# tpoisonooo/how-to-optimize-gemm

Measured on AMD Instinct MI355X. Metric: GFLOPS vs N (square SGEMM sweep); % of MI355X fp32 MFMA peak at N=4096, higher is better.
Workload: dtype f32; 1 GPU; sgemm fp32 square N=4096, 1xMI355X, kernel=auto (BASELINE configs[2]); m=4096, n=4096, k=4096, kernel=MMult_hip_auto, parallelism=single, rows_per_rank=4096

## Files before the change

### how-to-optimize-gemm_amd/csrc/abi.hip

```cpp
#include <algorithm>

#include "internal.hpp"
#include "igemm_plan.hpp"
#ifdef MMH_AB_BUILD
#include "ab_kernels.hpp"
#endif

using namespace mmh;

namespace {
template <typename F>
int time_calls(mmh_context *h, void *stream, int warmup, int reps, float *ms_per_call, const char *what, F call) {
  if (!h || reps <= 0 || warmup < 0 || !ms_per_call) return MMH_ERR_INVALID_ARG;
  ENTER(h);
  hipStream_t s = static_cast<hipStream_t>(stream);
  int rc = MMH_OK;
  for (int i = 0; i < warmup && rc == MMH_OK; ++i) rc = call(s);
  if (rc != MMH_OK) return rc;
  hipEvent_t t0 = nullptr, t1 = nullptr;
  hipError_t e = hipEventCreate(&t0);
  if (e == hipSuccess) e = hipEventCreate(&t1);
  if (e == hipSuccess) e = hipEventRecord(t0, s);
  for (int i = 0; i < reps && rc == MMH_OK && e == hipSuccess; ++i) rc = call(s);
  float ms = 0.f;
// ... 41 lines not shown
  return time_calls(h, stream, warmup, reps, ms_per_call, what, [&](hipStream_t s) {
    c.g.s = s;
    return call_on(h, c.call, h->kernel, c.g, c.b);
  });
}

constexpr KernelRow kKernels[] = {
    {MMH_KERNEL_AUTO, "MMult_hip_auto", Launcher::Auto, -1},
    {MMH_KERNEL_VALU, "MMult_hip_valu", Launcher::Valu, -1},
    {MMH_KERNEL_VALU_128X128, "MMult_hip_valu_128x128", Launcher::Valu, -1},
    {MMH_KERNEL_VALU_64X64, "MMult_hip_valu_64x64", Launcher::Valu, -1},
    {MMH_KERNEL_VALU_128X64, "MMult_hip_valu_128x64", Launcher::Valu, -1},
    {MMH_KERNEL_MFMA, "MMult_hip_mfma", Launcher::Reg, -1},
    {MMH_KERNEL_MFMA_256, "MMult_hip_mfma256", Launcher::Reg, -1},
    {MMH_KERNEL_NAIVE, "MMult_hip_naive", Launcher::Naive, -1},
    {MMH_KERNEL_MFMA_SIMPLE, "MMult_hip_mfma_simple", Launcher::Reg, -1},
    {MMH_KERNEL_MFMA_PIPE, "MMult_hip_mfma_pipe", Launcher::Reg, -1},
    {MMH_KERNEL_MFMA_TILES, "MMult_hip_mfma_tiles", Launcher::Reg, -1},
    {MMH_KERNEL_MFMA_128X64, "MMult_hip_mfma_128x64", Launcher::Reg, -1},
    {MMH_KERNEL_MFMA_64X64, "MMult_hip_mfma_64x64", Launcher::Reg, -1},
    {MMH_KERNEL_MFMA_256X256, "MMult_hip_mfma_256x256", Launcher::Reg, -1},
    {MMH_KERNEL_MFMA_64X64_DMA, "MMult_hip_mfma_64x64_dma", Launcher::K2L, MMH_KERNEL_MFMA_64X64},
    {MMH_KERNEL_MFMA_128X64_DMA, "MMult_hip_mfma_128x64_dma", Launcher::K2L, MMH_KERNEL_MFMA_128X64},
    {MMH_KERNEL_MFMA_128X128_DMA, "MMult_hip_mfma_128x128_dma", Launcher::K2L, MMH_KERNEL_MFMA},
    {MMH_KERNEL_MFMA_64X64_DMA5, "MMult_hip_mfma_64x64_dma5", Launcher::K2W, MMH_KERNEL_MFMA_64X64},
    {MMH_KERNEL_MFMA_128X64_DMA5, "MMult_hip_mfma_128x64_dma5", Launcher::K2W, MMH_KERNEL_MFMA_128X64},
    {MMH_KERNEL_MFMA_128X128_DMA5, "MMult_hip_mfma_128x128_dma5", Launcher::K2W, MMH_KERNEL_MFMA},
    {MMH_KERNEL_MFMA_96X96_DMA5, "MMult_hip_mfma_96x96_dma5", Launcher::K2W, MMH_KERNEL_MFMA},
    {MMH_KERNEL_MFMA_96X64_DMA5, "MMult_hip_mfma_96x64_dma5", Launcher::K2W, MMH_KERNEL_MFMA},
    {MMH_KERNEL_MFMA_160X160_DMA5, "MMult_hip_mfma_160x160_dma5", Launcher::K2W, MMH_KERNEL_MFMA},
    {MMH_KERNEL_MFMA_SPLITK, "MMult_hip_mfma_splitk", Launcher::SplitK, MMH_KERNEL_MFMA},
    {MMH_KERNEL_MFMA_SPLITK_128X64, "MMult_hip_mfma_splitk_128x64", Launcher::SplitK, MMH_KERNEL_MFMA_128X64},
#ifdef MMH_AB_BUILD
#include "ab_kernels.inc"
#endif
};
constexpr int kMaxKernelId = 127;
struct KernelIndex {
  signed char row[kMaxKernelId + 1];
  bool ok;
};
constexpr KernelIndex kernel_index() {
  KernelIndex ix{};
  ix.ok = true;
  for (signed char &r : ix.row) r = -1;
  int n = 0;
  for (const KernelRow &r : kKernels) {
    if (r.id < 0 || r.id > kMaxKernelId || ix.row[r.id] >= 0) ix.ok = false;
    else ix.row[r.id] = (signed char)n;
    ++n;
  }
  for (const KernelRow &r : kKernels)
    if (r.fallback >= 0 && (ix.row[r.fallback] < 0 || kKernels[ix.row[r.fallback]].launcher != Launcher::Reg)) ix.ok = false;
  return ix;
}
constexpr KernelIndex kKernelIndex = kernel_index();
static_assert(kKernelIndex.ok, "kKernels: an id twice or out of range, or a fall-back that is no register-staged id");

struct OptionRow {
  int id;
  int mmh_context::*field;
  int lo, hi;
  bool squash;
};
constexpr OptionRow kOptions[] = {
    {MMH_OPT_STREAMK, &mmh_context::streamk, 0, 2, false},
    {MMH_OPT_SPLITK, &mmh_context::splitk, 0, 16, false},
    {MMH_OPT_HOST_PANELS, &mmh_context::host_panels, -1, kMaxHostPanels, false},
    {MMH_OPT_STREAMK_ORDER, &mmh_context::sk_order, 0, 1, true},
    {MMH_OPT_STREAMK_CHAIN, &mmh_context::sk_chain, 0, 1, true},
    {MMH_OPT_PERSIST, &mmh_context::persist, 0, 1, false},
    {MMH_OPT_RIM, &mmh_context::rim, 0, kAbBuild ? 16 : 0, false},
    {MMH_OPT_RIM5, &mmh_context::rim5, 0, 0, kAbBuild},
#ifdef MMH_AB_BUILD
    {100, &mmh_context::pin, 0, 1, true},
    {101, &mmh_context::ab_group_m, 0, 1024, false},
    {102, &mmh_context::ab_nodefer, 0, 1, true},
    {103, &mmh_context::ab_own_occ, 0, 1, true},
    {104, &mmh_context::sk_order_min10, 10, 1000, false},
    {105, &mmh_context::ab_valu_old, 0, 1, true},
    {106, &mmh_context::ab_whole_ranges, 0, 1, true},
    {107, &mmh_context::split_tail, 0, 1, true},
    {108, &mmh_context::ab_batch_major, 0, 1, true},
#endif
};
const OptionRow *option_row(int option) {
  for (const OptionRow &r : kOptions)
    if (r.id == option) return &r;
  return nullptr;
}
}

const KernelRow *mmh::kernel_row(int kernel) {
  if (kernel < 0 || kernel > kMaxKernelId || kKernelIndex.row[kernel] < 0) return nullptr;
  return &kKernels[kKernelIndex.row[kernel]];
}

extern "C" {

const char *mmh_strerror(int status) {
  switch (status) {
    case MMH_OK: return "success";
    case MMH_ERR_INVALID_ARG: return "invalid argument";
    case MMH_ERR_HIP: return "HIP runtime error";
    case MMH_ERR_NO_DEVICE: return "no gfx950 device";
    case MMH_ERR_UNSUPPORTED: return "unsupported in this build";
    case MMH_ERR_ALLOC: return "allocation failed";
    case MMH_ERR_COMM: return "RCCL error";
    default: return "unknown status";
  }
}

const char *mmh_last_error(void) { return last_error_ref().c_str(); }

const char *mmh_last_launch(void) { return last_launch_ref().c_str(); }

int mmh_version(void) { return 303; }

int mmh_is_ab_build(void) {
#ifdef MMH_AB_BUILD
  return 1;
#else
  return 0;
#endif
}

int mmh_device_count(int *count) {
  if (!count) return MMH_ERR_INVALID_ARG;
  int c = 0;
  hipError_t e = hipGetDeviceCount(&c);
  if (e != hipSuccess) {
    *count = 0;
    (void)hipGetLastError();
    return MMH_OK;
  }
  *count = c;
  return MMH_OK;
}

int mmh_device_info(int device, char *name, int *cu_count, int *clock_mhz) {
  hipDeviceProp_t prop;
  HIP_TRY(hipGetDeviceProperties(&prop, device));
  if (name) snprintf(name, 256, "%s (%s)", prop.name, prop.gcnArchName);
  if (cu_count) *cu_count = prop.multiProcessorCount;
  if (clock_mhz) *clock_mhz = prop.clockRate / 1000;
  return MMH_OK;
}

int mmh_create(mmh_handle_t *handle, int device) {
  if (!handle) return MMH_ERR_INVALID_ARG;
  return create_context(handle, device);
}

int mmh_destroy(mmh_handle_t h) {
  destroy_context(h);
  return MMH_OK;
}

int mmh_set_kernel(mmh_handle_t h, int kernel) {
  if (!h || !known_kernel(kernel)) return MMH_ERR_INVALID_ARG;
  h->kernel = kernel;
  return MMH_OK;
}

int mmh_set_option(mmh_handle_t h, int option, int value) {
  if (!h) return MMH_ERR_INVALID_ARG;
// ... 240 lines not shown
```

### how-to-optimize-gemm_amd/csrc/internal.hpp

```cpp
#pragma once
#include <hip/hip_runtime.h>
#include <stdint.h>
#include <stdio.h>
#include <string.h>

#include <initializer_list>
#include <string>
#include <utility>
#include <vector>

#include "ab_build.hpp"
#include "../../include/mmult_hip.h"

namespace mmh {

void set_last_error(const std::string &s);
void set_last_launch(const std::string &s);
const std::string &last_error_ref();
const std::string &last_launch_ref();
int hip_fail(hipError_t e, const char *what);

#define HIP_TRY(expr)                                        \
  do {                                                       \
    hipError_t e_ = (expr);                                  \
// ... 27 lines not shown
struct GemmArgs {
  int m, n, k;
  const float *A;
  int lda;
  const float *B;
  int ldb;
  float *C;
  int ldc;
  int acc;
  hipStream_t s;
  int rim_m = 0, rim_n = 0;
  int form = 0;
  int sk_w = 0;
  int ta = 0, tb = 0;
  int ex = 0;
  float alpha = 1.0f, beta = 0.0f;
  const float *bias = nullptr;
  int bias_mode = MMH_BIAS_NONE, act = MMH_ACT_NONE;
};
inline GemmArgs op_args(int ta, int tb, int m, int n, int k, const float *dA, int lda, const float *dB, int ldb, float *dC, int ldc,
                        int accumulate, hipStream_t s) {
  GemmArgs g{m, n, k, dA, lda, dB, ldb, dC, ldc, accumulate ? 1 : 0, s};
  g.ta = ta;
  g.tb = tb;
  return g;
}
inline GemmArgs ex_args_of(GemmArgs g, float alpha, float beta, const float *dBias, int bias_mode, int activation) {
  g.acc = 0;
  g.ex = 1;
  g.alpha = alpha;
  g.beta = beta;
  g.bias = dBias;
  g.bias_mode = bias_mode;
  g.act = activation;
  return g;
}

}

struct mmh_context {
  int device = 0;
  int kernel = MMH_KERNEL_AUTO;
  int cu_count = 0;
  mmh::DevBuf a, b, c;
  mmh::Scratch bt;
  int igemm_mode = 0;
  int i8_grid_cap = 0;
  mmh::Scratch qa, qb, qc, qs;
  void *qs_zeros_of = nullptr;
  mmh::Scratch colsum_parts;
  struct StreamWs {
    hipStream_t stream = nullptr;
    mmh::DevBuf flags;
    bool flags_dirty = true;
    mmh::DevBuf parts;
    unsigned long stamp = 0;
    bool captured = false;
  };
  std::vector<StreamWs *> ws;
  unsigned long ws_stamp = 0;
  int *sk_stats = nullptr;
  std::vector<void *> retired;
  int streamk = 1;
  int splitk = 0;
  int host_panels = -1;
  void *rocblas = nullptr;
  void *blaslt = nullptr;
  int *sticky = nullptr;
  int *sticky_dev = nullptr;
  long long spin_limit = 1ll << 26;
  int fault = 0;
  int pin = 1;
  int sk_order = 1;
  int sk_order_min10 = 18;
  int dma_edge = 1;
  int dma_dword_rows = 1;
  int sk_chain = 1;
  int rim5 = 0;
  int ab_whole_ranges = 0;
  int ab_nodefer = 0;
  int ab_valu_old = 0;
  int ab_own_occ = 0;
  int split_tail = 1;
  int ab_group_m = 0;
  int ab_batch_major = 0;
  int persist = 0;
  int rim = 0;
  struct SkTable {
    long tiles = 0;
    int nk = 0, grid = 0;
    mmh::DevBuf buf;
    int *host = nullptr;
    size_t host_ints = 0;
    unsigned long stamp = 0;
    bool pinned = false;
    bool uploaded = false;
    std::vector<hipStream_t> upload_streams;
  };
  std::vector<SkTable *> sk_tables;
  unsigned long sk_stamp = 0;
  std::vector<std::pair<const void *, int>> per_cu;
  bool warmed = false;
  hipStream_t hs_in = nullptr, hs_run = nullptr, hs_out = nullptr;
  hipEvent_t ev_in[mmh::kMaxHostPanels] = {}, ev_run[mmh::kMaxHostPanels] = {}, ev_b = nullptr;
  bool pipeline_ready = false;
  hipEvent_t t0 = nullptr, t1 = nullptr;
};

namespace mmh {

int check_sticky(mmh_context *h);
#define ENTER(h)                                       \
  ::mmh::DeviceGuard guard_;                           \
  HIP_TRY(guard_.enter((h)->device));                  \
  if (int st_ = ::mmh::check_sticky(h); st_ != MMH_OK) return st_

int create_context(mmh_context **out, int device, bool warm = true);
void destroy_context(mmh_context *h);
int warm_context(mmh_context *h);

inline bool aligned16(const void *p) { return (reinterpret_cast<uintptr_t>(p) & 15) == 0; }
inline bool capturing(hipStream_t s) {
  hipStreamCaptureStatus cap = hipStreamCaptureStatusNone;
  (void)hipStreamIsCapturing(s, &cap);
  return cap != hipStreamCaptureStatusNone;
}

inline bool fast_shape(int BM, int BN, int KB, const GemmArgs &g) {
  return (g.m % BM == 0) && (g.n % BN == 0) && (g.k % KB == 0) && (g.lda % 4 == 0) && (g.ldb % 4 == 0) &&
         (g.ldc % 4 == 0) && aligned16(g.A) && aligned16(g.B) && aligned16(g.C);
}
inline bool window_ok(int BM, int BN, int k, int lda, int ldb) {
  const size_t lim = (1ull << 31) - 4096;
  return ((size_t)BM * lda + k) * 4 < lim && ((size_t)k * ldb + BN) * 4 < lim;
}
inline bool window_ok(int BM, int BN, const GemmArgs &g) {
  if (!g.ta && !g.tb) return window_ok(BM, BN, g.k, g.lda, g.ldb);
  const size_t lim = (1ull << 31) - 4096;
  const size_t a = g.ta ? (size_t)g.k * g.lda + BM : (size_t)BM * g.lda + g.k;
  const size_t b = g.tb ? (size_t)BN * g.ldb + g.k : (size_t)g.k * g.ldb + BN;
  return a * 4 < lim && b * 4 < lim;
}

int check_gemm_args(int m, int n, int k, const void *A, int lda, const void *B, int ldb, const void *C, int ldc, int ta = 0,
                    int tb = 0);

enum class Launcher { Auto, Valu, Naive, Reg, SplitK, K2L, K2W, K2M  };
struct KernelRow {
  int id;
  const char *name;
  Launcher launcher;
  int fallback;
};
const KernelRow *kernel_row(int kernel);
inline bool known_kernel(int kernel) { return kernel_row(kernel) != nullptr; }
inline bool is_family(int kernel, Launcher l) {
  const KernelRow *r = kernel_row(kernel);
  return r && r->launcher == l;
}

int workspace_for(mmh_context *ctx, hipStream_t s, long tiles, size_t parts_bytes, int **flags, float **parts);
int reserve_stream(mmh_context *ctx, hipStream_t s, int m, int n, int k);
void workspaces_suspect(mmh_context *ctx);
int reserve_scratch(mmh_context *ctx, hipStream_t s, const char *who, std::initializer_list<ScratchNeed> needs);
bool build_sk_tables(long tiles, int nk, int grid, int *order, int *place);
int sk_tables_for(mmh_context *ctx, long tiles, int nk, int grid, hipStream_t s, const int **order, const int **place, int min10 = 0);

int auto_plan(int m, int n, int k, int lda, int ldb, int ldc, int base_align, int cu_count, int *kernel, long *tiles,
              int *streamk_grid);
int sgemm_on(mmh_context *ctx, int kernel, int m, int n, int k, const float *dA, int lda, const float *dB, int ldb,
             float *dC, int ldc, int accumulate, hipStream_t s);
int auto_plan_op(int ta, int tb, int m, int n, int k, int lda, int ldb, int ldc, int base_align, int cu_count, int *kernel,
                 long *tiles, int *streamk_grid, int ex = 0);
int launch_reg(mmh_context *ctx, int kernel, const GemmArgs &g);
int launch_reg_splitk(mmh_context *ctx, int tile , int S, const GemmArgs &g);
int warm_reg(mmh_context *ctx, float *scratch, hipStream_t s);
int launch_dma(mmh_context *ctx, int kernel, const GemmArgs &g);
bool dma_shape_ok(const mmh_context *ctx, int kernel, const GemmArgs &g);
int warm_dma(mmh_context *ctx, float *scratch, hipStream_t s);
int launch_dma32(mmh_context *ctx, int kernel, const GemmArgs &g);
bool dma32_shape_ok(const mmh_context *ctx, int kernel, const GemmArgs &g);
int warm_dma32(mmh_context *ctx, float *scratch, hipStream_t s);
inline bool dma5_tail_split(long tiles, long w, long cus, int k) {
  const long rem = tiles - w * cus;
  return w >= 2 && k >= 512 && 100 * rem > 85 * cus && rem <= cus && (w * cus) % 8 == 0;
}

inline bool dma5_rim_dims(int m, int n, int *r_m, int *r_n) {
  const int rm = m % 64, rn = n % 64;
  const int a = (rm == 1 && m > 64) ? 1 : 0, b = (rn == 1 && n > 64) ? 1 : 0;
  if (r_m) *r_m = a;
  if (r_n) *r_n = b;
  return a > 0 || b > 0;
}
template <class... Tile>
struct TileTable {
  template <class F>
  static int with(int kernel, F &&f, int none) {
    int r = none;
    (void)((kernel == Tile::ID && ((r = f(Tile{})), true)) || ...);
    return r;
  }
  template <class F>
  static int each(F &&f) {
    int rc = MMH_OK;
    (void)(((rc = f(Tile{})) == MMH_OK) && ...);
    return rc;
  }
};

template <int ID_, int BM_, int BN_, int WTN_, int WTM_, int KB_>
struct RegTile {
  static constexpr int ID = ID_, BM = BM_, BN = BN_, WTN = WTN_, WTM = WTM_, KB = KB_;
};
using reg_tiles = TileTable<
    RegTile<MMH_KERNEL_MFMA,         128, 128, 4, 4, 32>,
    RegTile<MMH_KERNEL_MFMA_256X256, 256, 256, 4, 8, 32>,
    RegTile<MMH_KERNEL_MFMA_128X64,  128, 64,  2, 4, 32>,
    RegTile<MMH_KERNEL_MFMA_64X64,   64,  64,  2, 2, 128>>;
inline long reg_tile_count(int kernel, int m, int n) {
  long tiles = 0;
  reg_tiles::with(kernel, [&](auto t) {
    tiles = (long)((m + t.BM - 1) / t.BM) * ((n + t.BN - 1) / t.BN);
    return 0;
  }, 0);
  return tiles;
}

template <int ID_, int BM_, int BN_, int KB_, int WTM_, int WTN_, int NBUF_>
struct K2lTile {
  static constexpr int ID = ID_, BM = BM_, BN = BN_, KB = KB_, WTM = WTM_, WTN = WTN_, NBUF = NBUF_;
};
using k2l_tiles = TileTable<
    K2lTile<MMH_KERNEL_MFMA_64X64_DMA,   64,  64,  32, 2, 2, 3>,
    K2lTile<MMH_KERNEL_MFMA_128X64_DMA,  128, 64,  32, 4, 2, 3>,
    K2lTile<MMH_KERNEL_MFMA_128X128_DMA, 128, 128, 32, 4, 4, 3>>;

template <int ID_, int BM_, int BN_, int WTM_, int WTN_, int NBUF_, int NL_, int D_, bool SK_, bool OPS_, int RS_ = 1>
struct K2wTile {
  static constexpr int ID = ID_, BM = BM_, BN = BN_, WTM = WTM_, WTN = WTN_, NBUF = NBUF_, NL = NL_, D = D_, RS = RS_;
  static constexpr bool SK = SK_, OPS = OPS_;
};
#define MMH_K2W_ARGS(K) K::BM, K::BN, 32, K::WTM, K::WTN, K::NBUF
using k2w_tiles = TileTable<
    K2wTile<MMH_KERNEL_MFMA_64X64_DMA5,   64,  64, 2, 2, 3, 2, 2, true,  true>,
    K2wTile<MMH_KERNEL_MFMA_128X64_DMA5,  128, 64, 4, 2, 3, 4, 2, true,  true>,
    K2wTile<MMH_KERNEL_MFMA_128X128_DMA5, 128, 128, 4, 4, 3, 4, 2, true, true>,
    K2wTile<MMH_KERNEL_MFMA_96X96_DMA5,   96,  96, 3, 3, 3, 1, 2, false, false>,
    K2wTile<MMH_KERNEL_MFMA_160X160_DMA5, 160, 160, 5, 5, 3, 4, 2, false, false>,
    K2wTile<MMH_KERNEL_MFMA_96X64_DMA5,   96,  64, 3, 2, 3, 4, 2, false, false>>;

struct BatchArgs {
  long long sA = 0, sB = 0, sC = 0;
  long batch = 1;
  long long sBias = 0;
};
constexpr long kBatchedMaxWorkgroups = MMH_BATCHED_MAX_WORKGROUPS;

inline int dma5_form(const mmh_context *ctx, int BM, int BN, const GemmArgs &g, const BatchArgs &b = BatchArgs{}) {
  if (!window_ok(BM, BN, g)) return -1;
  const bool s4 = b.batch == 1 || (b.sA % 4 == 0 && b.sB % 4 == 0 && b.sC % 4 == 0);
  if (fast_shape(BM, BN, 32, g) && s4) return 0;
  if (!ctx || !ctx->dma_edge) return -1;
  const bool rows16 = (g.lda % 4 == 0) && (g.ldb % 4 == 0) && aligned16(g.A) && aligned16(g.B) &&
                      (b.batch == 1 || (b.sA % 4 == 0 && b.sB % 4 == 0));
  if (!rows16 && !ctx->dma_dword_rows) return -1;
  return 1;
}
// ... 51 lines not shown
```

### how-to-optimize-gemm_amd/csrc/launch_dma5.hpp

```cpp
#pragma once
#include <stdarg.h>

#include <tuple>

#include "ab_build.hpp"
#include "launch_common.hpp"
#include "sgemm_dma5.hpp"

namespace mmh {

inline const char *op_tag(const GemmArgs &g) {
  return g.ta ? (g.tb ? ", operands TT" : ", operands TN") : (g.tb ? ", operands NT" : "");
}
inline std::string ex_tag(const GemmArgs &g) {
  std::string t = std::string(g.ta ? (g.tb ? ", operands TT" : ", operands TN") : (g.tb ? ", operands NT" : ", operands NN")) + ", epilogue";
  const size_t bare = t.size();
  if (g.alpha != 1.0f) t += " alpha";
  if (g.beta != 0.0f) t += " beta";
  if (g.bias_mode == MMH_BIAS_COL) t += " bias(col)";
  if (g.bias_mode == MMH_BIAS_ROW) t += " bias(row)";
  if (g.act == MMH_ACT_RELU) t += " relu";
  if (t.size() == bare) t += " identity";
  return t;
}
inline Dma5Epilogue ex_args(const GemmArgs &g) { return Dma5Epilogue{g.alpha, g.beta, g.bias, g.bias_mode, g.act}; }

template <typename K>
long dma5_split_first(mmh_context *ctx, K twin, int threads, size_t lds, long tiles, int k) {
  if (!ctx || !ctx->split_tail) return tiles;
  (void)allow_big_lds(twin, lds);
  const long cus = ctx->cu_count > 0 ? ctx->cu_count : 256;
  const long w = std::min(resident_per_cu(ctx, twin, threads, lds), 3);
  return dma5_tail_split(tiles, w, cus, k) ? w * cus : tiles;
}

template <class K_>
struct NnForm {
  using K = K_;
  static constexpr bool NN = true, SK = K::SK;
  static constexpr const char *plain_name = "sgemm_mfma_dma5_kernel", *streamk_name = "sgemm_dma5_streamk_kernel";
  static auto plain(bool edge) {
    return edge ? sgemm_mfma_dma5_kernel<MMH_K2W_ARGS(K), true, K::NL, K::D, K::RS>
                : sgemm_mfma_dma5_kernel<MMH_K2W_ARGS(K), false, K::NL, K::D, K::RS>;
  }
  static auto streamk_bound() { return sgemm_dma5_streamk_kernel<MMH_K2W_ARGS(K), true, true, K::NL, K::D, K::RS>; }
  static auto streamk(bool edge, bool chained) {
    return edge ? (chained ? streamk_bound() : sgemm_dma5_streamk_kernel<MMH_K2W_ARGS(K), true, false, K::NL, K::D, K::RS>)
                : (chained ? sgemm_dma5_streamk_kernel<MMH_K2W_ARGS(K), false, true, K::NL, K::D, K::RS>
                           : sgemm_dma5_streamk_kernel<MMH_K2W_ARGS(K), false, false, K::NL, K::D, K::RS>);
  }
  static std::string tag(const GemmArgs &) { return {}; }
  static std::tuple<> extra(const GemmArgs &) { return {}; }
  static int acc(const mmh_context *ctx, const GemmArgs &g) {
    if (kAbBuild && ctx) return g.acc | (ctx->ab_nodefer ? 2 : 0) | (ctx->ab_whole_ranges ? 4 : 0) | ((ctx->ab_group_m & 0xff) << 8);
    return g.acc;
  }
};
template <class K_, int OP>
struct OpForm {
  using K = K_;
  static constexpr bool NN = false, SK = K::SK;
  static constexpr const char *plain_name = "sgemm_mfma_dma5_op_kernel", *streamk_name = "sgemm_dma5_op_streamk_kernel";
  static auto plain(bool edge) {
    return edge ? sgemm_mfma_dma5_op_kernel<MMH_K2W_ARGS(K), true, K::NL, K::D, OP>
                : sgemm_mfma_dma5_op_kernel<MMH_K2W_ARGS(K), false, K::NL, K::D, OP>;
  }
  static auto streamk(bool edge, bool) {
    return edge ? sgemm_dma5_op_streamk_kernel<MMH_K2W_ARGS(K), true, K::NL, K::D, OP>
                : sgemm_dma5_op_streamk_kernel<MMH_K2W_ARGS(K), false, K::NL, K::D, OP>;
  }
  static std::string tag(const GemmArgs &g) { return op_tag(g); }
  static std::tuple<> extra(const GemmArgs &) { return {}; }
  static int acc(const mmh_context *, const GemmArgs &g) { return g.acc; }
};
template <class K_, int OP>
struct ExForm {
  using K = K_;
  static constexpr bool NN = false, SK = K::SK;
  static constexpr const char *plain_name = "sgemm_mfma_dma5_ex_kernel", *streamk_name = "sgemm_dma5_ex_streamk_kernel";
  static auto plain(bool edge) {
    return edge ? sgemm_mfma_dma5_ex_kernel<MMH_K2W_ARGS(K), true, K::NL, K::D, OP>
                : sgemm_mfma_dma5_ex_kernel<MMH_K2W_ARGS(K), false, K::NL, K::D, OP>;
  }
  static auto streamk(bool edge, bool) {
    return edge ? sgemm_dma5_ex_streamk_kernel<MMH_K2W_ARGS(K), true, K::NL, K::D, OP>
                : sgemm_dma5_ex_streamk_kernel<MMH_K2W_ARGS(K), false, K::NL, K::D, OP>;
  }
  static std::string tag(const GemmArgs &g) { return ex_tag(g); }
  static std::tuple<Dma5Epilogue> extra(const GemmArgs &g) { return {ex_args(g)}; }
  static int acc(const mmh_context *, const GemmArgs &) { return 0; }
};

template <class K_, int OP>
struct BatchedForm {
  using K = K_;
  static constexpr bool SK = false;
  static constexpr const char *plain_name = "sgemm_mfma_dma5_batched_kernel";
  static auto plain(bool edge) {
    return edge ? sgemm_mfma_dma5_batched_kernel<MMH_K2W_ARGS(K), true, K::NL, K::D, OP>
                : sgemm_mfma_dma5_batched_kernel<MMH_K2W_ARGS(K), false, K::NL, K::D, OP>;
  }
  static std::string tag(const GemmArgs &g) { return op_tag(g); }
  static std::tuple<int> front(const mmh_context *ctx, const GemmArgs &g) {
    return {g.acc | ((kAbBuild && ctx && ctx->ab_batch_major) ? 2 : 0)};
  }
  static std::tuple<> back(const GemmArgs &, const BatchArgs &, long) { return {}; }
};
inline std::tuple<Dma5Epilogue, long long> ex_chunk_args(const GemmArgs &g, const BatchArgs &bt, long b0) {
  const bool none = g.bias_mode == MMH_BIAS_NONE;
  Dma5Epilogue ep = ex_args(g);
  ep.bias = none ? nullptr : g.bias + b0 * bt.sBias;
  return {ep, none ? 0 : bt.sBias};
}
template <class K_, int OP>
struct BatchedExForm {
  using K = K_;
  static constexpr bool SK = false;
  static constexpr const char *plain_name = "sgemm_mfma_dma5_batched_ex_kernel";
  static auto plain(bool edge) {
    return edge ? sgemm_mfma_dma5_batched_ex_kernel<MMH_K2W_ARGS(K), true, K::NL, K::D, OP>
                : sgemm_mfma_dma5_batched_ex_kernel<MMH_K2W_ARGS(K), false, K::NL, K::D, OP>;
  }
  static std::string tag(const GemmArgs &g) { return ex_tag(g); }
  static std::tuple<> front(const mmh_context *, const GemmArgs &) { return {}; }
  static std::tuple<Dma5Epilogue, long long> back(const GemmArgs &g, const BatchArgs &bt, long b0) { return ex_chunk_args(g, bt, b0); }
};

constexpr int kTextSize = 448;
inline int text_add(char *what, int at, const char *format, ...) __attribute__((format(printf, 3, 4)));
inline int text_add(char *what, int at, const char *format, ...) {
  va_list args;
  va_start(args, format);
  const int n = vsnprintf(what + at, kTextSize - at, format, args);
  va_end(args);
  return std::min(at + std::max(n, 0), kTextSize - 1);
}
template <class K>
int dma5_tile_text(char *what, const char *kernel) {
  return text_add(what, 0, "%s<%d,%d> wave tile %dx%d, K-slice %d x %d ring buffers by %d loader wave%s' LDS-DMA, fragments %d k-steps ahead",
                  kernel, K::BM, K::BN, 16 * K::WTM, 16 * K::WTN, 32, K::NBUF, K::NL, K::NL > 1 ? "s" : "", K::D);
}
template <class K>
int dma5_plain_text(char *what, const char *kernel, bool edge, long workgroups, bool split) {
  return text_add(what, dma5_tile_text<K>(what, kernel), ", %s%ld workgroups of %d threads%s", edge ? "guarded, " : "", workgroups,
                  Dma5Tile<MMH_K2W_ARGS(K), K::NL>::THREADS, split ? " (the last round as a launch of its own)" : "");
}
template <class L>
void dma5_launch_rounds(long first, long tiles, L launch) {
  launch(first, 0L);
  if (first < tiles) launch(tiles - first, first);
}

template <class F>
int launch_dma5_tile(mmh_context *ctx, const GemmArgs &g) {
  using K = typename F::K;
  constexpr int BM = K::BM, BN = K::BN, KB = 32;
  using T = Dma5Tile<MMH_K2W_ARGS(K), K::NL>;
  const int form = dma5_form(ctx, BM, BN, g);
  if (form < 0) return 1;
  const bool edge = form == 1;
  GemmArgs ga = g;
  ga.acc = F::acc(ctx, g);
  if constexpr (F::SK) {
    if (ctx && ctx->streamk) {
      const bool chained = !F::NN || ctx->sk_chain != 0;
      auto occ = NnForm<K>::streamk_bound();
      auto kern = F::streamk(edge, chained);
      if constexpr (F::NN) {
        if (kAbBuild && ctx->ab_own_occ && !edge) occ = kern;
      } else {
        (void)allow_big_lds(occ, T::LDS_BYTES);
      }
      char what[kTextSize];
      text_add(what, dma5_tile_text<K>(what, F::streamk_name), "%s%s", chained ? ", chained parts" : "", edge ? ", guarded" : "");
      const int order_min10 = (BM == 128 && BN == 128) ? 10 : 0;
      const int sk = std::apply([&](auto... x) {
        return launch_streamk(ctx, kern, occ, BM, BN, KB, T::THREADS, T::LDS_BYTES, what, ga, full_tiles(g.m, g.n, BM, BN), order_min10, x...);
      }, F::extra(g));
      if (!F::NN && sk == MMH_OK) set_last_launch(last_launch_ref() + F::tag(g));
      if (sk <= 0) return sk;
    }
  }
  const int nbm = (g.m + BM - 1) / BM, nbn = (g.n + BN - 1) / BN;
  const long tiles = (long)nbm * nbn;
  const long first = dma5_split_first(ctx, NnForm<K>::plain(edge), T::THREADS, T::LDS_BYTES, tiles, g.k);
  const int acc_bits = edge ? F::acc(nullptr, g) : ga.acc;
  auto kern = F::plain(edge);
  const int ok = allow_big_lds(kern, T::LDS_BYTES);
  if (ok != MMH_OK) return ok;
  dma5_launch_rounds(first, tiles, [&](long workgroups, long id0) {
    std::apply([&](auto... x) {
      hipLaunchKernelGGL(kern, dim3((unsigned)workgroups), dim3(T::THREADS), T::LDS_BYTES, g.s, g.m, g.n, g.k, g.A, g.lda, g.B, g.ldb, g.C,
                         g.ldc, acc_bits | (int)((unsigned)(id0 >> 3) << 16), nbm, nbn, x...);
    }, F::extra(g));
  });
  HIP_TRY(hipGetLastError());
  char what[kTextSize];
  text_add(what, dma5_plain_text<K>(what, F::plain_name, edge, tiles, first < tiles), "%s", F::tag(g).c_str());
  set_last_launch(what);
  return MMH_OK;
}

template <class F>
int launch_batched_tile(mmh_context *ctx, const GemmArgs &g, const BatchArgs &bt) {
  using K = typename F::K;
  using T = Dma5Tile<MMH_K2W_ARGS(K), K::NL>;
  const int form = dma5_form(ctx, K::BM, K::BN, g, bt);
  if (form < 0) return 1;
  const bool edge = form == 1;
  auto kern = F::plain(edge);
  const int ok = allow_big_lds(kern, T::LDS_BYTES);
  if (ok != MMH_OK) return ok;
  const int nbm = (g.m + K::BM - 1) / K::BM, nbn = (g.n + K::BN - 1) / K::BN;
  const long per = (long)nbm * nbn;
  const long mats = std::max(1L, kBatchedMaxWorkgroups / per);
  long launches = 0;
  bool split = false;
  for (long b0 = 0; b0 < bt.batch; b0 += mats) {
    const long tiles = std::min(mats, bt.batch - b0) * per;
    const float *A = g.A + b0 * bt.sA, *B = g.B + b0 * bt.sB;
    float *C = g.C + b0 * bt.sC;
    const long first = dma5_split_first(ctx, NnForm<K>::plain(edge), T::THREADS, T::LDS_BYTES, tiles, g.k);
    dma5_launch_rounds(first, tiles, [&](long workgroups, long id0) {
      std::apply([&](auto... x) {
        hipLaunchKernelGGL(kern, dim3((unsigned)workgroups), dim3(T::THREADS), T::LDS_BYTES, g.s, g.m, g.n, g.k, A, g.lda, bt.sA, B, g.ldb,
                           bt.sB, C, g.ldc, bt.sC, x...);
      }, std::tuple_cat(F::front(ctx, g), std::make_tuple(nbm, nbn, (unsigned)id0), F::back(g, bt, b0)));
      ++launches;
    });
    split |= first < tiles;
    HIP_TRY(hipGetLastError());
  }
  char what[kTextSize];
  int at = dma5_plain_text<K>(what, F::plain_name, edge, bt.batch * per, split);
  at = text_add(what, at, "%s, batch %ld", F::tag(g).c_str(), bt.batch);
  if (launches > 1) text_add(what, at, " as %ld launches", launches);
  set_last_launch(what);
  return MMH_OK;
}

template <class L>
int launch_naive_chunks(const GemmArgs &g, const BatchArgs &b, std::string what, L launch) {
  const long gx = (g.n + 63) / 64, gy = (g.m + 3) / 4;
  const long mats = std::max(1L, std::min(65535L, kBatchedMaxWorkgroups / (gx * gy)));
  long launches = 0;
  for (long b0 = 0; b0 < b.batch; b0 += mats) {
    launch(dim3((unsigned)gx, (unsigned)gy, (unsigned)std::min(mats, b.batch - b0)), g.A ? g.A + b0 * b.sA : nullptr,
           g.B ? g.B + b0 * b.sB : nullptr, g.C + b0 * b.sC, b0);
    ++launches;
    HIP_TRY(hipGetLastError());
  }
  what += ", batch " + std::to_string(b.batch);
  if (launches > 1) what += " as " + std::to_string(launches) + " launches";
  set_last_launch(what);
  return MMH_OK;
}

template <template <class, int> class F, int... OPS, class L>
int launch_form(int kernel, const GemmArgs &g, L launch) {
  const int op = g.ta | (g.tb << 1);
  return k2w_tiles::with(kernel, [&](auto t) {
    using K = decltype(t);
    int rc = 1;
    if constexpr (K::OPS) {
      auto launch_if = [&](auto form, int form_op) {
        if (op == form_op) rc = launch(form);
      };
      (launch_if(F<K, OPS>{}, OPS), ...);
    }
    return rc;
  }, 1);
}
template <class F>
int warm_form_tile() {
  constexpr size_t lds = Dma5Tile<MMH_K2W_ARGS(F::K), F::K::NL>::LDS_BYTES;
  int rc;
  if ((rc = allow_big_lds(F::plain(false), lds)) != MMH_OK || (rc = allow_big_lds(F::plain(true), lds)) != MMH_OK) return rc;
  if constexpr (F::SK)
    if ((rc = allow_big_lds(F::streamk(false, true), 160 * 1024)) == MMH_OK) rc = allow_big_lds(F::streamk(true, true), 160 * 1024);
  return rc;
}
// ... 17 lines not shown
```

### how-to-optimize-gemm_amd/csrc/sgemm_dma5.hpp

```cpp
#pragma once
#include <type_traits>

#include "ab_build.hpp"
#include "sgemm_dma.hpp"
#include "sgemm_mfma.hpp"

namespace mmh {

constexpr int dma5_gcd(int a, int b) { return b == 0 ? a : dma5_gcd(b, a % b); }

template <int BM, int BN, int KB, int WTM, int WTN, int NBUF, int NL = 1>
struct Dma5Tile {
  static_assert(KB == 32, "a K-slice row of A is 128 bytes: a piece of A is eight rows");
  static_assert(BM == 32 * WTM && BN == 32 * WTN, "four consumer waves as 2 x 2, wave tile 16 WTM x 16 WTN");
  static_assert(WTM >= 2 && WTM <= 6 && WTN >= 2 && WTN <= 6, "wave tile 32 .. 96 rows / columns");
  static_assert(NBUF >= 2 && NBUF <= 6, "ring depth (2: the next slice is requested after barrier kt - 1 and waited for before barrier kt -- K1W's two co-resident workgroups)");
  static_assert(NL == 1 || NL == 2 || NL == 4, "one, two or four loader waves");
  static constexpr int CONSUMERS = 4, LOADER = 4;
  static constexpr int WAVES_M = 2, WAVES_N = 2;
  static constexpr int THREADS = 64 * (CONSUMERS + NL);
  static constexpr bool BBLK = (WTN % 2) != 0;
  static constexpr int A_FLOATS = BM * KB, B_FLOATS = KB * BN, STAGE = A_FLOATS + B_FLOATS, KS = KB / 4;
  static constexpr int CHA = A_FLOATS / 256, CHB = B_FLOATS / 256, NP = CHA + CHB;
  static constexpr int NPL = NP / NL;
// ... 629 lines not shown
            }
            if constexpr (CHAIN) __builtin_amdgcn_sched_barrier(0);
          }
        return;
      }
    }
    auto out_vec = [&](int t, int r) {
      bfrag_t v;
#pragma unroll
      for (int u = 0; u < WTN; ++u) v[u] = u < NU ? acc[t][u < NU ? u : 0][r] : 0.0f;
      return v;
    };
    if (part_out) {
      __amdgpu_buffer_rsrc_t rsrc_p;
      if constexpr (PART_WT) rsrc_p = __builtin_amdgcn_make_buffer_rsrc(part_out, 0, BM * BN * 4, 0x00020000);
#pragma unroll
      for (int t = 0; t < NT; ++t)
#pragma unroll
        for (int r = 0; r < 4; ++r) {
          const int row = crow + 16 * t + r;
          const bfrag_t v = out_vec(t, r);
          const uint32_t off = (uint32_t)(((row - row0) * BN + (ccol - col0)) * 4);
          if constexpr (!VEC) {
#pragma unroll
            for (int u = 0; u < NU; ++u) {
              constexpr int STEP = BBLK ? 16 : 1;
              if constexpr (PART_WT) __builtin_amdgcn_raw_buffer_store_b32(__builtin_bit_cast(int, (float)v[u]), rsrc_p, off + 4u * STEP * u, 0, 16);
              else part_out[(size_t)(row - row0) * BN + (ccol - col0) + STEP * u] = v[u];
            }
          } else if constexpr (PART_WT) {
            if constexpr (WTN == 4) {
              typedef int i32x4_t __attribute__((ext_vector_type(4)));
              __builtin_amdgcn_raw_buffer_store_b128(__builtin_bit_cast(i32x4_t, v), rsrc_p, off, 0, 16);
            } else {
              static_assert(!VEC || WTN == 2 || WTN == 4 || !PART_WT, "write-through partial tiles: 8- or 16-byte vectors");
              typedef int i32x2_t __attribute__((ext_vector_type(2)));
              __builtin_amdgcn_raw_buffer_store_b64(__builtin_bit_cast(i32x2_t, v), rsrc_p, off, 0, 16);
            }
          } else {
            *reinterpret_cast<bfrag_t *>(part_out + (size_t)(row - row0) * BN + (ccol - col0)) = v;
          }
        }
    } else if (VEC && whole_c) {
      if constexpr (VEC) {
#pragma unroll
        for (int t = 0; t < NT; ++t)
#pragma unroll
          for (int r = 0; r < 4; ++r) *reinterpret_cast<c_vec *>(C + (size_t)(crow + 16 * t + r) * ldc + ccol) = out_vec(t, r);
      }
    } else {
#pragma unroll
      for (int t = 0; t < NT; ++t)
#pragma unroll
        for (int r = 0; r < 4; ++r) {
          const int row = crow + 16 * t + r;
          const bfrag_t v = out_vec(t, r);
          if (whole_c || row < m) {
#pragma unroll
            for (int u = 0; u < NU; ++u)
              if (whole_c || col_of(u) < n) C[(size_t)row * ldc + col_of(u)] = v[u];
          }
        }
    }
  }
};

template <int BM, int BN, bool EDGE>
__device__ __forceinline__ void dma5_raster(int bid, int m, int n, int nbm, int nbn, int gm, int &tm, int &tn) {
  const int thin_row = (EDGE && nbm > 1 && m - (nbm - 1) * BM <= 16) ? 1 : 0, thin_col = (EDGE && nbn > 1 && n - (nbn - 1) * BN <= 16) ? 1 : 0;
  const int n_full = (nbm - thin_row) * (nbn - thin_col);
  int r = bid - n_full;
  if (r < 0) {
    block_to_tile_g(bid, n_full, nbm - thin_row, nbn - thin_col, gm, tm, tn);
  } else if (thin_col && r < nbm) {
    tm = r;
    tn = nbn - 1;
  } else {
    if (thin_col) r -= nbm;
    tm = nbm - 1;
    tn = r;
  }
}

template <int BM, int BN, int KB, int WTM, int WTN, int NBUF, bool EDGE = false, int NL = 1, int D = 2, int RS = 1>
__global__ void __launch_bounds__(64 * (4 + NL))
sgemm_mfma_dma5_kernel(int m, int n, int k, const float *__restrict__ A, int lda, const float *__restrict__ B, int ldb,
                       float *__restrict__ C, int ldc, int accumulate, int nbm, int nbn) {
  extern __shared__ __attribute__((aligned(16))) float lds[];
  using S = Dma5Segment<BM, BN, KB, WTM, WTN, NBUF, false, EDGE, false, NL, D, false, false, RS>;
  constexpr int GM = Dma5Tile<BM, BN, KB, WTM, WTN, NBUF, NL>::GM;
  int tm, tn;
  asm volatile("" ::"s"(A), "s"(B), "s"(C), "s"(lda), "s"(ldb), "s"(ldc), "s"(k));
  dma_stamp(0);
  const unsigned bid = blockIdx.x + (((unsigned)accumulate >> 16) << 3);
  accumulate &= 0xffff;
  if constexpr (EDGE) {
    dma5_raster<BM, BN, true>(bid, m, n, nbm, nbn, GM, tm, tn);
  } else {
    int gm = GM;
    if constexpr (kAbBuild) {
      const int ab_gm = (accumulate >> 8) & 0xff;
      accumulate &= 1;
      if (ab_gm > 0) gm = ab_gm;
    }
    block_to_tile_g(bid, nbm * nbn, nbm, nbn, gm, tm, tn);
  }
  typename S::Lane L;
  L.init(lda, ldb);
  typename S::Frags fr;
  Dma5Link link;
  int no_reply = 0;
  S::run(lds, L, m, n, k, A, lda, B, ldb, C, ldc, tm, tn, 0, (k + KB - 1) / KB, accumulate != 0, nullptr, nullptr, fr, link,
         Dma5Next{}, nullptr, no_reply);
  dma_stamp_after_stores(3);
}

template <int BM, int BN, int KB, int WTM, int WTN, int NBUF, bool EDGE, int NL, int D, int OP>
__global__ void __launch_bounds__(64 * (4 + NL))
sgemm_mfma_dma5_op_kernel(int m, int n, int k, const float *__restrict__ A, int lda, const float *__restrict__ B, int ldb,
                          float *__restrict__ C, int ldc, int accumulate, int nbm, int nbn) {
  extern __shared__ __attribute__((aligned(16))) float lds[];
  using S = Dma5Segment<BM, BN, KB, WTM, WTN, NBUF, false, EDGE, false, NL, D, false, false, 1, OP>;
  constexpr int GM = Dma5Tile<BM, BN, KB, WTM, WTN, NBUF, NL>::GM;
  asm volatile("" ::"s"(A), "s"(B), "s"(C), "s"(lda), "s"(ldb), "s"(ldc), "s"(k));
  const unsigned bid = blockIdx.x + (((unsigned)accumulate >> 16) << 3);
  accumulate &= 0xffff;
  int tm, tn;
  dma5_raster<BM, BN, EDGE>(bid, m, n, nbm, nbn, GM, tm, tn);
  typename S::Lane L;
  L.init(lda, ldb);
  typename S::Frags fr;
  Dma5Link link;
  int no_reply = 0;
  S::run(lds, L, m, n, k, A, lda, B, ldb, C, ldc, tm, tn, 0, (k + KB - 1) / KB, accumulate != 0, nullptr, nullptr, fr, link,
         Dma5Next{}, nullptr, no_reply);
}

template <int BM, int BN, int KB, int WTM, int WTN, int NBUF, bool EDGE, int NL, int D, int OP>
__global__ void __launch_bounds__(64 * (4 + NL))
sgemm_mfma_dma5_batched_kernel(int m, int n, int k, const float *__restrict__ A, int lda, long long sA,
                               const float *__restrict__ B, int ldb, long long sB, float *__restrict__ C, int ldc,
                               long long sC, int accumulate, int nbm, int nbn, unsigned first) {
  extern __shared__ __attribute__((aligned(16))) float lds[];
  using S = Dma5Segment<BM, BN, KB, WTM, WTN, NBUF, false, EDGE, false, NL, D, false, false, 1, OP>;
  constexpr int GM = Dma5Tile<BM, BN, KB, WTM, WTN, NBUF, NL>::GM;
  asm volatile("" ::"s"(A), "s"(B), "s"(C), "s"(lda), "s"(ldb), "s"(ldc), "s"(k));
  bool xcd_runs = true;
  if constexpr (kAbBuild) {
    xcd_runs = (accumulate & 2) == 0;
    accumulate &= 1;
  }
  const unsigned G = gridDim.x, x = blockIdx.x;
  unsigned id = x;
  if (xcd_runs) {
    const unsigned xcd = x % NXCD, local = x / NXCD, q = G / NXCD, r = G % NXCD;
    id = (xcd < r ? xcd * (q + 1) : r * (q + 1) + (xcd - r) * q) + local;
  }
  id += first;
  const unsigned per = (unsigned)nbm * (unsigned)nbn;
  const unsigned b = id / per;
  const int bid = (int)(id - b * per);
  A += (long long)b * sA;
  B += (long long)b * sB;
  C += (long long)b * sC;
  int tm, tn;
  const int thin_row = (EDGE && nbm > 1 && m - (nbm - 1) * BM <= 16) ? 1 : 0, thin_col = (EDGE && nbn > 1 && n - (nbn - 1) * BN <= 16) ? 1 : 0;
  const int n_full = (nbm - thin_row) * (nbn - thin_col);
  int r = bid - n_full;
  if (r < 0) {
    block_to_tile_g(bid, n_full, nbm - thin_row, nbn - thin_col, GM, tm, tn);
  } else if (thin_col && r < nbm) {
    tm = r;
    tn = nbn - 1;
  } else {
    if (thin_col) r -= nbm;
    tm = nbm - 1;
    tn = r;
  }
  typename S::Lane L;
  L.init(lda, ldb);
  typename S::Frags fr;
  Dma5Link link;
  int no_reply = 0;
  S::run(lds, L, m, n, k, A, lda, B, ldb, C, ldc, tm, tn, 0, (k + KB - 1) / KB, accumulate != 0, nullptr, nullptr, fr, link,
         Dma5Next{}, nullptr, no_reply);
}


// ... 311 lines not shown
```

Measured before the change: 151,700 GFLOPS.

## Walk multiple tiles per resident workgroup with cross-tile prefetch in dma5 kernel

Adds a persistent-style mode for the 128x128 dma5 kernel. When the tile count is an exact multiple of the resident grid, each workgroup loops over its tiles, using a lane-held tile table and passing the next tile to the segment so its loads can start before the current tile finishes. This targets per-tile launch and pipeline ramp-up and drain costs. The price is a new kernel path, more code size, and possible register pressure.

```diff
diff --git a/how-to-optimize-gemm_amd/csrc/abi.hip b/how-to-optimize-gemm_amd/csrc/abi.hip
--- a/how-to-optimize-gemm_amd/csrc/abi.hip
+++ b/how-to-optimize-gemm_amd/csrc/abi.hip
@@ -147,6 +147,7 @@
     {106, &mmh_context::ab_whole_ranges, 0, 1, true},
     {107, &mmh_context::split_tail, 0, 1, true},
     {108, &mmh_context::ab_batch_major, 0, 1, true},
+    {109, &mmh_context::walk_rounds, 0, 2, false},
 #endif
 };
 const OptionRow *option_row(int option) {
diff --git a/how-to-optimize-gemm_amd/csrc/internal.hpp b/how-to-optimize-gemm_amd/csrc/internal.hpp
--- a/how-to-optimize-gemm_amd/csrc/internal.hpp
+++ b/how-to-optimize-gemm_amd/csrc/internal.hpp
@@ -133,6 +133,7 @@
   int ab_valu_old = 0;
   int ab_own_occ = 0;
   int split_tail = 1;
+  int walk_rounds = 1;
   int ab_group_m = 0;
   int ab_batch_major = 0;
   int persist = 0;
@@ -235,6 +236,10 @@
 inline bool dma5_tail_split(long tiles, long w, long cus, int k) {
   const long rem = tiles - w * cus;
   return w >= 2 && k >= 512 && 100 * rem > 85 * cus && rem <= cus && (w * cus) % 8 == 0;
+}
+inline bool dma5_walk_rounds(long tiles, long w, long cus, int k, int nbuf) {
+  const long grid = w * cus;
+  return grid > 0 && grid % 8 == 0 && tiles % grid == 0 && tiles / grid >= 2 && tiles / grid <= 63 && k / 32 >= nbuf - 1;
 }
 
 inline bool dma5_rim_dims(int m, int n, int *r_m, int *r_n) {
diff --git a/how-to-optimize-gemm_amd/csrc/launch_dma5.hpp b/how-to-optimize-gemm_amd/csrc/launch_dma5.hpp
--- a/how-to-optimize-gemm_amd/csrc/launch_dma5.hpp
+++ b/how-to-optimize-gemm_amd/csrc/launch_dma5.hpp
@@ -32,6 +32,15 @@
   const long cus = ctx->cu_count > 0 ? ctx->cu_count : 256;
   const long w = std::min(resident_per_cu(ctx, twin, threads, lds), 3);
   return dma5_tail_split(tiles, w, cus, k) ? w * cus : tiles;
+}
+template <typename K>
+long dma5_walk_grid(mmh_context *ctx, K kern, bool product, int threads, size_t lds, int nbm, int nbn, int k, int nbuf) {
+  if (!ctx || ctx->walk_rounds < (product ? 1 : 2) || nbm >= 32768 || nbn >= 32768) return 0;
+  const long tiles = (long)nbm * nbn;
+  (void)allow_big_lds(kern, lds);
+  const long cus = ctx->cu_count > 0 ? ctx->cu_count : 256;
+  const long w = std::min(resident_per_cu(ctx, kern, threads, lds), 3);
+  return dma5_walk_rounds(tiles, w, cus, k, nbuf) ? w * cus : 0;
 }
 
 template <class K_>
@@ -184,11 +193,16 @@
   const int nbm = (g.m + BM - 1) / BM, nbn = (g.n + BN - 1) / BN;
   const long tiles = (long)nbm * nbn;
   const long first = dma5_split_first(ctx, NnForm<K>::plain(edge), T::THREADS, T::LDS_BYTES, tiles, g.k);
-  const int acc_bits = edge ? F::acc(nullptr, g) : ga.acc;
+  int acc_bits = edge ? F::acc(nullptr, g) : ga.acc;
   auto kern = F::plain(edge);
   const int ok = allow_big_lds(kern, T::LDS_BYTES);
   if (ok != MMH_OK) return ok;
-  dma5_launch_rounds(first, tiles, [&](long workgroups, long id0) {
+  long walk = 0;
+  if constexpr (F::NN && K::SK && dma5_walk_tile(BM, BN)) {
+    if (!edge && first == tiles) walk = dma5_walk_grid(ctx, kern, BM == 128 && BN == 128, T::THREADS, T::LDS_BYTES, nbm, nbn, g.k, K::NBUF);
+  }
+  if (walk > 0) acc_bits |= kDma5WalkBit;
+  dma5_launch_rounds(walk > 0 ? walk : first, walk > 0 ? walk : tiles, [&](long workgroups, long id0) {
     std::apply([&](auto... x) {
       hipLaunchKernelGGL(kern, dim3((unsigned)workgroups), dim3(T::THREADS), T::LDS_BYTES, g.s, g.m, g.n, g.k, g.A, g.lda, g.B, g.ldb, g.C,
                          g.ldc, acc_bits | (int)((unsigned)(id0 >> 3) << 16), nbm, nbn, x...);
@@ -196,7 +210,9 @@
   });
   HIP_TRY(hipGetLastError());
   char what[kTextSize];
-  text_add(what, dma5_plain_text<K>(what, F::plain_name, edge, tiles, first < tiles), "%s", F::tag(g).c_str());
+  int at = dma5_plain_text<K>(what, F::plain_name, edge, tiles, first < tiles);
+  if (walk > 0) at = text_add(what, at, ", walked by %ld resident workgroups, %ld tiles each", walk, tiles / walk);
+  text_add(what, at, "%s", F::tag(g).c_str());
   set_last_launch(what);
   return MMH_OK;
 }
diff --git a/how-to-optimize-gemm_amd/csrc/sgemm_dma5.hpp b/how-to-optimize-gemm_amd/csrc/sgemm_dma5.hpp
--- a/how-to-optimize-gemm_amd/csrc/sgemm_dma5.hpp
+++ b/how-to-optimize-gemm_amd/csrc/sgemm_dma5.hpp
@@ -735,6 +735,11 @@
   }
 }
 
+constexpr bool dma5_walk_tile(int BM, int BN) {
+  return (BM == 128 && BN == 128) || (kAbBuild && ((BM == 64 && BN == 64) || (BM == 128 && BN == 64)));
+}
+constexpr int kDma5WalkBit = 8;
+
 template <int BM, int BN, int KB, int WTM, int WTN, int NBUF, bool EDGE = false, int NL = 1, int D = 2, int RS = 1>
 __global__ void __launch_bounds__(64 * (4 + NL))
 sgemm_mfma_dma5_kernel(int m, int n, int k, const float *__restrict__ A, int lda, const float *__restrict__ B, int ldb,
@@ -742,6 +747,7 @@
   extern __shared__ __attribute__((aligned(16))) float lds[];
   using S = Dma5Segment<BM, BN, KB, WTM, WTN, NBUF, false, EDGE, false, NL, D, false, false, RS>;
   constexpr int GM = Dma5Tile<BM, BN, KB, WTM, WTN, NBUF, NL>::GM;
+  constexpr bool WALK = !EDGE && dma5_walk_tile(BM, BN);
   int tm, tn;
   asm volatile("" ::"s"(A), "s"(B), "s"(C), "s"(lda), "s"(ldb), "s"(ldc), "s"(k));
   dma_stamp(0);
@@ -751,12 +757,51 @@
     dma5_raster<BM, BN, true>(bid, m, n, nbm, nbn, GM, tm, tn);
   } else {
     int gm = GM;
+    const bool walk = WALK && (accumulate & kDma5WalkBit) != 0;
+    if constexpr (WALK) accumulate &= ~kDma5WalkBit;
     if constexpr (kAbBuild) {
       const int ab_gm = (accumulate >> 8) & 0xff;
       accumulate &= 1;
       if (ab_gm > 0) gm = ab_gm;
     }
     block_to_tile_g(bid, nbm * nbn, nbm, nbn, gm, tm, tn);
+    if constexpr (WALK) {
+      if (walk) {
+        using SW = Dma5Segment<BM, BN, KB, WTM, WTN, NBUF, false, false, true, NL, D, false, false, RS>;
+        const int tiles = nbm * nbn, nk = k / KB;
+        int tab = -1;
+        {
+          const int v = (int)bid + (int)(threadIdx.x & 63) * (int)gridDim.x;
+          if (v < tiles) {
+            int ltm, ltn;
+            block_to_tile_g(v, tiles, nbm, nbn, gm, ltm, ltn);
+            tab = ltm | (ltn << 16);
+          }
+        }
+        typename SW::Lane LW;
+        LW.init(lda, ldb);
+        typename SW::Frags frw;
+        Dma5Link linkw;
+        int no_reply_w = 0;
+        auto walk_tiles = [&]() {
+          for (int i = 0;; ++i) {
+            const int cur = __builtin_amdgcn_readlane(tab, i), nxt = __builtin_amdgcn_readlane(tab, i + 1);
+            Dma5Next nx;
+            if (nxt >= 0) {
+              nx.tm = nxt & 0xffff;
+              nx.tn = nxt >> 16;
+              nx.len = nk;
+            }
+            SW::run(lds, LW, m, n, k, A, lda, B, ldb, C, ldc, cur & 0xffff, cur >> 16, 0, nk, accumulate != 0, nullptr, nullptr, frw,
+                    linkw, nx, nullptr, no_reply_w);
+            if (nxt < 0) break;
+          }
+        };
+        if (LW.loader) walk_tiles();
+        else walk_tiles();
+        return;
+      }
+    }
   }
   typename S::Lane L;
   L.init(lda, ldb);
```

New measurement: 152,000 GFLOPS (median of 2 runs). About the same (+0.2%).
